# bbc/turingcodec

Hardware: AMD Instinct MI355X
Metric: encoded fps (havoc hot path, primitive-batch throughput: one picture's primitive calls per frame as whole-frame batches; (higher is better)
Workload: dtype u8

## Files before the change

### turingcodec_amd/csrc/kernels_rdoq.hip

```cpp
#include "common.h"
#include "rdoq_work.h"

#include <cstdlib>

namespace havoc_gpu {

#ifdef HAVOC_RDOQ_TIMING
__device__ unsigned long long g_rdoqTiming[32];
struct RdoqTimer
{
    unsigned long long acc[16] = {}, last = __builtin_readcyclecounter();
    __device__ __forceinline__ void mark(int k)
    {
        const unsigned long long now = __builtin_readcyclecounter();
        acc[k] += now - last;
        last = now;
    }
    __device__ __forceinline__ void flush(int lane, int base)
    {
        if (lane != 0) return;
        for (int k = 0; k < 16; ++k)
            if (acc[k]) atomicAdd(&g_rdoqTiming[base + k], acc[k]);
    }
};
#define RT_DECL RdoqTimer rt
#define RT_MARK(k) rt.mark(k)
#define RT_PARAM , RdoqTimer &rt
#define RT_ARG , rt
#define RT_FLUSH(lane, base) rt.flush(lane, base)
#else
#define RT_DECL
#define RT_MARK(k)
#define RT_PARAM
#define RT_ARG
#define RT_FLUSH(lane, base)
#endif

namespace {

__device__ const int32_t kEntropyBits[128] = {
    0x07b23, 0x085f9, 0x074a0, 0x08cbc, 0x06ee4, 0x09354, 0x067f4, 0x09c1b, 0x060b0, 0x0a62a, 0x05a9c, 0x0af5b, 0x0548d, 0x0b955, 0x04f56, 0x0c2a9,
    0x04a87, 0x0cbf7, 0x045d6, 0x0d5c3, 0x04144, 0x0e01b, 0x03d88, 0x0e937, 0x039e0, 0x0f2cd, 0x03663, 0x0fc9e, 0x03347, 0x10600, 0x03050, 0x10f95,
    0x02d4d, 0x11a02, 0x02ad3, 0x12333, 0x0286e, 0x12cad, 0x02604, 0x136df, 0x02425, 0x13f48, 0x021f4, 0x149c4, 0x0203e, 0x1527b, 0x01e4d, 0x15d00,
    0x01c99, 0x166de, 0x01b18, 0x17017, 0x019a5, 0x17988, 0x01841, 0x18327, 0x016df, 0x18d50, 0x015d9, 0x19547, 0x0147c, 0x1a083, 0x0138e, 0x1a8a3,
    0x01251, 0x1b418, 0x01166, 0x1bd27, 0x01068, 0x1c77b, 0x00f7f, 0x1d18e, 0x00eda, 0x1d91a, 0x00e19, 0x1e254, 0x00d4f, 0x1ec9a, 0x00c90, 0x1f6e0,
    0x00c01, 0x1fef8, 0x00b5f, 0x208b1, 0x00ab6, 0x21362, 0x00a15, 0x21e46, 0x00988, 0x2285d, 0x00934, 0x22ea8, 0x008a8, 0x239b2, 0x0081d, 0x24577,
    0x007c9, 0x24ce6, 0x00763, 0x25663, 0x00710, 0x25e8f, 0x006a0, 0x26a26, 0x00672, 0x26f23, 0x005e8, 0x27ef8, 0x005ba, 0x284b5, 0x0055e, 0x29057,
    0x0050c, 0x29bab, 0x004c1, 0x2a674, 0x004a7, 0x2aa5e, 0x0046f, 0x2b32f, 0x0041f, 0x2c0ad, 0x003e7, 0x2ca8d, 0x003ba, 0x2d323, 0x0010c, 0x3bfbb };

typedef short s16x2v __attribute__((ext_vector_type(2)));
typedef unsigned short u16x2v __attribute__((ext_vector_type(2)));

static_assert(sizeof(havoc_mi355x_rdoq_job) == sizeof(RdoqJob), "rdoq job layout");

struct Block
{
    const uint8_t *states;
    const int32_t *bits;
    const int32_t *lastBits;
    int stateStride, lastStride, lastLen;
    int64_t lambda;
    int distShift;
    int quantScale, quantShift, invScale, invShift, invOffset;
    int cIdx, scanIdx;
    uint64_t scan4;
    int64_t csbfZero[2], csbfOne[2];
    int64_t cbfZero, cbfOne;
    const uint32_t *clsTab;
};

struct LevelState { int ctxSet, c1, nG1, nG2, rice; };

__device__ __forceinline__ int32_t bitsOf(const Block &b, int ctx, int bin) { return b.bits[(b.states[ctx * b.stateStride] >> 1) ^ bin]; }
template <class T>
__device__ __forceinline__ T pick(bool c, T a, T b) { return c ? a : b; }

__device__ __forceinline__ int baseLevel(const LevelState &s) { return pick(s.nG1 < 8, 2 + (int)(s.nG2 < 1), 1); }
__device__ __forceinline__ int clip16(int v) { return min(max(v, -32768), 32767); }

__device__ __forceinline__ void diagXy(int size, int pos, int &x, int &y)
{
    for (int d = 0;; ++d)
    {
        const int lo = d < size ? 0 : d - size + 1, hi = d < size ? d : size - 1, len = hi - lo + 1;
        if (pos < len) { x = lo + pos; y = d - x; return; }
        pos -= len;
    }
}
__device__ __forceinline__ void scanXy(int size, int scanIdx, int pos, int &x, int &y)
{
    if (scanIdx == 1) { x = pos & (size - 1); y = pos / size; }
    else if (scanIdx == 2) { x = pos / size; y = pos & (size - 1); }
    else diagXy(size, pos, x, y);
}
__host__ __device__ constexpr uint64_t scan4Nibbles(int scanIdx)
{
    uint64_t v = 0;
    int i = 0;
    if (scanIdx == 0)
    {
        for (int d = 0; d < 7; ++d)
            for (int x = 0; x <= d; ++x)
                if (x < 4 && d - x < 4) { v |= (uint64_t)(x | (d - x) << 2) << (4 * i); ++i; }
    }
    else
        for (; i < 16; ++i) v |= (uint64_t)(scanIdx == 1 ? i : (i >> 2) | (i & 3) << 2) << (4 * i);
    return v;
}

template <int GW>
__device__ __forceinline__ void toScanOrder(int scanIdx, uint64_t &m, uint64_t &m2, uint64_t &m3)
{
    if (GW == 1 || scanIdx == 1) return;
    uint64_t a = 0, b = 0, c = 0;
    int x = 0, y = 0;
    for (int g = 0; g < GW * GW; ++g)
    {
        const int p = y * GW + x;
        a |= ((m >> p) & 1) << g;
        b |= ((m2 >> p) & 1) << g;
        c |= ((m3 >> p) & 1) << g;
        if (scanIdx == 2)
        {
            if (++y == GW) { y = 0; ++x; }
        }
        else
// ... 200 lines not shown
            z = bitsOf(b, ctx, 0);
            one = bitsOf(b, ctx, 1);
            zeroBits += pick(inside & !nonZero, z, 0);
        }
        else
        {
            const bool is1 = (cls1 >> i) & 1, is2 = (cls2 >> i) & 1, isD = i == 0 && dcGroup;
            z = pick(isD, zcD, pick(is1, zc1, pick(is2, zc2, zc0)));
            one = pick(isD, ocD, pick(is1, oc1, pick(is2, oc2, oc0)));
        }
        sh.rec.kept[nib][lane] = 0;
        const int32_t upZero = (int32_t)((uint32_t)factor * (uint32_t)-(scaled >> (b.quantShift - 8))) + (1 << 15) + one - z;
        sh.rec.costUp[i][lane] = pick(inside, upZero, 1 << 15);
    }
    const uint32_t zeroMask = active & ~nzMask;
    if (LOG2 > 2)
        zeroBits = zc0 * __popc(zeroMask & cls0) + zc1 * __popc(zeroMask & cls1) + zc2 * __popc(zeroMask & cls2) + zcD * __popc(zeroMask & clsD);
    const int64_t sumSq = ((int64_t)sumAllHi << 16) + sumAll;
    r.dist0 = sumSq << b.distShift;

    RT_MARK(4);
    int nonZeroAbovePos0 = 0;
    int64_t gSig = 0, gSigPos0 = 0, gCoded = 0, gDist0 = 0, costB = 0, distB = 0, qB = 0;
    uint32_t c1At = 0x55555555u;
    uint32_t keptMask = 0, oddMask = 0;
    for (uint32_t m = nzMask; m;)
    {
        const int i = 31 - __clz((int)m);
        m ^= 1u << i;
        const int nib = (int)(b.scan4 >> (4 * i)) & 15, x = (gx << 2) + (nib & 3), y = (gy << 2) + (nib >> 2);
        const int a = abs((int)sh.coef[nib][lane]);
        const int64_t dist0 = (int64_t)(a * a) << b.distShift;
        const int sp = g * 16 + i;
        const int scaled = a * b.quantScale;
        const int level = (scaled + rnd) >> b.quantShift;
        const bool first = sp == firstPos;
        int32_t z0, z1, aboveBits;
        if (LOG2 == 2)
        {
            const uint32_t pk = reinterpret_cast<const uint32_t (*)[64]>(sh.rec.costDown)[i][lane];
            const int sc = (int)(pk >> 25);
            aboveBits = (int32_t)(pk & 0x1ffffff);
            z0 = bitsOf(b, sc, 0);
            z1 = bitsOf(b, sc, 1);
        }
        else
        {
            const bool is1 = (cls1 >> i) & 1, is2 = (cls2 >> i) & 1, isD = (clsD >> i) & 1;
            z0 = pick(isD, zcD, pick(is1, zc1, pick(is2, zc2, zc0)));
            z1 = pick(isD, ocD, pick(is1, oc1, pick(is2, oc2, oc0)));
            const uint32_t above = zeroMask & ~((2u << i) - 1);
            aboveBits = zc0 * __popc(above & cls0) + zc1 * __popc(above & cls1) + zc2 * __popc(above & cls2);
        }
        const int64_t zerosAbove = b.lambda * aboveBits;
        const int32_t sigZero = pick(first, 0, z0), sigOneBits = pick(first, 0, z1);
        fb.g1zero = pick4(aux.g1zero, st.c1);
        fb.g1one = pick4(g1one, st.c1);

        const bool droppable = !first && level < 3;
        const int64_t sigOne = b.lambda * sigOneBits, dropSig = b.lambda * sigZero;
        const int lower = level - 1;
        const int32_t err1 = a - clip16((clip16(level) * b.invScale + b.invOffset) >> b.invShift);
        const int32_t err2 = a - clip16((clip16(lower) * b.invScale + b.invOffset) >> b.invShift);
        const int64_t cost1 = ((int64_t)(int32_t)((uint32_t)err1 * (uint32_t)err1) << b.distShift) + b.lambda * levelBits(level, st, fb) + sigOne;
        const int64_t cost2If = ((int64_t)(int32_t)((uint32_t)err2 * (uint32_t)err2) << b.distShift) + b.lambda * levelBits(lower, st, fb) + sigOne;
        const int64_t cost2 = pick(lower >= 1, cost2If, (int64_t)INT64_MAX);
        const int64_t dropCost = dist0 + dropSig;
        int64_t costCoded = pick(droppable, dropCost, (int64_t)INT64_MAX), costSig = pick(droppable, dropSig, (int64_t)0);
        int kept = 0;
        const bool take1 = cost1 < costCoded;
        kept = pick(take1, level, kept);
        costSig = pick(take1, sigOne, costSig);
        costCoded = pick(take1, cost1, costCoded);
        const bool take2 = cost2 < costCoded;
        kept = pick(take2, lower, kept);
        costSig = pick(take2, sigOne, costSig);
        costCoded = pick(take2, cost2, costCoded);

        costB += costCoded;
        distB += dist0;
        const int du = (scaled - (kept << b.quantShift)) >> (b.quantShift - 8), sigDelta = sigOneBits - sigZero;
        const int stored = (int16_t)kept;
        const int now = levelRate(kept, st, fb);
        const int upKept = factor * -du + levelRate(kept + 1, st, fb) - now;
        const int upZero = factor * -abs(du) + (1 << 15) + sigDelta;
        sh.rec.kept[nib][lane] = (int16_t)kept;
        keptMask |= (uint32_t)(stored != 0) << i;
        oddMask |= (uint32_t)(stored & 1) << i;
        sh.rec.costUp[i][lane] = pick(kept > 0, upKept, upZero);
        const int lastOne = (1 << 15) + sigDelta;
        sh.rec.costDown[i][lane] = factor * du + levelRate(kept - 1, st, fb) - now - pick(kept == 1, lastOne, 0);

        const bool grow = (kept >= baseLevel(st)) & (kept > 3 * (1 << st.rice));
        st.rice = pick(grow, min(st.rice + 1, 4), st.rice);
        st.nG1 += kept >= 1;
        st.nG2 += kept > 1;
        const bool step = (st.c1 < 3) & (st.c1 > 0) & (kept != 0);
        st.c1 = pick(kept > 1, 0, pick(step, st.c1 + 1, st.c1));
        {
            const uint32_t below = (1u << (2 * i)) - 1;
            c1At = (c1At & ~below) | ((0x55555555u * (uint32_t)st.c1) & below);
        }
        gSig += costSig;
        gSigPos0 = pick(i == 0, costSig, gSigPos0);
        const int64_t codedPart = costCoded - costSig;
        gCoded += pick(stored != 0, codedPart, (int64_t)0);
        gDist0 += pick(stored != 0, dist0, (int64_t)0);
        nonZeroAbovePos0 += (stored != 0) & (i != 0);
        const int lx = lastPrefixLength(x), ly = lastPrefixLength(y);
        const int32_t rate = b.lastBits[(b.scanIdx == 2 ? ly : lx) * b.lastStride] + b.lastBits[(b.lastLen + (b.scanIdx == 2 ? lx : ly)) * b.lastStride];
        const int64_t total = qB - zerosAbove + b.lambda * rate - costSig;
        const bool better = (stored != 0) & !r.localStop & (total < r.localBest);
        r.localBest = pick(better, total, r.localBest);
        r.localPos = pick(better, sp, r.localPos);
        r.localOr = pick(better, 0, r.localOr) | stored;
        r.groupOr |= stored;
        r.localStop |= stored > 1;
        const int64_t keptGain = dist0 - costCoded, zeroGain = -costSig;
        qB += pick(stored != 0, keptGain, zeroGain);
    }
    RT_MARK(5);
    aux.c1At = c1At;
    aux.keptMask = keptMask;
    aux.oddMask = oddMask;
    aux.negScan = negScan;
    aux.negRaster = negRaster;
    const int64_t zeroCost = b.lambda * zeroBits;
    r.cost = (r.dist0 - distB) + zeroCost + costB;
    r.q = qB - zeroCost;
    gSig += zeroCost;
    if (!(nzMask & 1))
        gSigPos0 = LOG2 == 2 ? zeroCost - b.lambda * (int32_t)(reinterpret_cast<const uint32_t (*)[64]>(sh.rec.costDown)[0][lane] & 0x1ffffff) : b.lambda * pick(dcGroup, zcD, pick((bool)(cls1 & 1), zc1, pick((bool)(cls2 & 1), zc2, zc0)));
    r.carry = st.c1 == 0;
    const bool dc = g == 0, any = keptMask != 0, inner = any & !dc & (g < firstGroup);
    const int64_t zero = pick(neighbours != 0, b.csbfZero[1], b.csbfZero[0]), one = pick(neighbours != 0, b.csbfOne[1], b.csbfOne[0]);
    const int64_t implied = pick(inner & (nonZeroAbovePos0 == 0), gSigPos0, (int64_t)0);
    const int64_t sigLeft = gSig - implied, allZero = zero + gDist0 - gCoded - sigLeft;
    const bool dropped = inner & (allZero < one), empty = !any & !dc;
    const int64_t innerCost = pick(dropped, allZero, one) - implied, emptyCost = zero - gSig;
    r.cost += pick(empty, emptyCost, pick(inner, innerCost, (int64_t)0));
    r.sigCost = pick(empty | dropped, zero, pick(inner, one, (int64_t)0));
    r.coded = dc | (any & !dropped);
    RT_MARK(6);
    return r;
}

__device__ __forceinline__ void hideSignsWalk(WalkShared &sh, int lane, const Block &b, bool lastGroup, const SdhAux &aux, uint32_t keptMask)
{
    const int first = max(__ffs((int)keptMask) - 1, 0), last = keptMask ? 31 - __clz((int)keptMask) : 0;
    const int signbit = (int)(aux.negScan >> first) & 1;
    const bool needed = (keptMask != 0) & (last - first >= 4) & (signbit != (__popc(aux.oddMask & keptMask) & 1));
    if (__ballot(needed) == 0) return;
    const int top = lastGroup ? last : 15;
    int minCost = INT32_MAX, minIdx = 0, finalChange = 0;
#pragma unroll
    for (int i = 15; i >= 0; --i)
    {
        const bool isKept = (keptMask >> i) & 1;
        const int mag = (uint16_t)sh.rec.kept[(int)(b.scan4 >> (4 * i)) & 15][lane];
        const int up = sh.rec.costUp[i][lane];
        const int downRaw = pick(isKept, sh.rec.costDown[i][lane], 0);
        const int down = downRaw - pick(lastGroup & (last == i) & (mag == 1), 4 << 15, 0);
        const bool upBetter = up < down;
        const int costKept = pick(upBetter, up, pick((i == first) & (mag == 1), INT32_MAX, down));
        const int g1 = pick((aux.active >> i) & 1, pick4(aux.g1zero, (int)(aux.c1At >> (2 * i)) & 3), 0);
        const int costZero = pick((i < first) & (((int)(aux.negScan >> i) & 1) != signbit), INT32_MAX, up + g1);
        const int cost = pick(isKept, costKept, costZero), change = pick(isKept & !upBetter, -1, 1);
        const bool better = (i <= top) & (cost < minCost);
        minCost = pick(better, cost, minCost);
        finalChange = pick(better, change, finalChange);
        minIdx = pick(better, i, minIdx);
    }
    if (!needed) return;
    const int nib = (int)(b.scan4 >> (4 * minIdx)) & 15;
    const int mag = (uint16_t)sh.rec.kept[nib][lane], negative = (int)(aux.negScan >> minIdx) & 1;
    if ((!negative && mag == 32767) || (negative && mag == 32768)) finalChange = -1;
    sh.rec.kept[nib][lane] = (int16_t)(mag + finalChange);
}

struct ScanShared
{
    int32_t srcOff[64], dstOff[64], nzThreshold[64], gt1Threshold[64], gt2Threshold[64];
    uint64_t mask[64], mask2[64], mask3[64];
    int64_t sumSq[64];
};
// ... 62 lines not shown
}

constexpr int kScanSteps = 8;
template <int LOG2>
__global__ __launch_bounds__(64) void k_rdoq_scan(int16_t *__restrict__ dstAll, const int16_t *__restrict__ srcAll, const RdoqJob *__restrict__ jobs, int njobs,
                                                  RdoqWork *__restrict__ work, int withHist)
{
    constexpr int perWg = kScanSteps * (64 / (((1 << LOG2) * (1 << LOG2)) >> 4));
    __shared__ ScanShared sc;
    __shared__ uint32_t hist[kBins];
    const int lane = threadIdx.x, first = blockIdx.x * perWg, blk = first + lane;
    RdoqInfo *info = reinterpret_cast<RdoqInfo *>(reinterpret_cast<char *>(work) + rdoqInfoOffset());
    for (int k = lane; k < kBins; k += 64) hist[k] = 0;
    scanBlocks<LOG2>(sc, dstAll, srcAll, jobs, njobs, first, kScanSteps);
    if (lane < perWg && blk < njobs)
    {
        RdoqInfo r;
        r.mask = sc.mask[lane];
        r.mask2 = sc.mask2[lane];
        r.mask3 = sc.mask3[lane];
        r.sumSq = sc.sumSq[lane];
        info[blk] = r;
        atomicAdd(&hist[groupsToWalk(r.mask)], 1u);
        if (jobs[blk].scan_idx != 0) atomicAdd(&hist[kBins - 1], 1u);
    }
    __syncthreads();
    if (!withHist) return;
    for (int k = lane; k < kBins - 1; k += 64)
        if (hist[k]) atomicAdd(&work->hist[k], hist[k]);
    if (lane == 0 && hist[kBins - 1]) atomicAdd(&work->otherScans, hist[kBins - 1]);
}

__global__ __launch_bounds__(256) void k_rdoq_hist(const RdoqJob *__restrict__ jobs, int njobs, RdoqWork *__restrict__ work)
{
    __shared__ uint32_t hist[kBins];
    const RdoqInfo *info = reinterpret_cast<const RdoqInfo *>(reinterpret_cast<const char *>(work) + rdoqInfoOffset());
    const int t = threadIdx.x, blk = blockIdx.x * 256 + t;
    if (t < kBins) hist[t] = 0;
    __syncthreads();
    if (blk < njobs)
    {
        atomicAdd(&hist[groupsToWalk(info[blk].mask)], 1u);
        if (jobs[blk].scan_idx != 0) atomicAdd(&hist[kBins - 1], 1u);
    }
    __syncthreads();
    if (t < kBins - 1 && hist[t]) atomicAdd(&work->hist[t], hist[t]);
    if (t == kBins - 1 && hist[t]) atomicAdd(&work->otherScans, hist[t]);
}

template <int LOG2>
__global__ __launch_bounds__(256) void k_rdoq_order(const RdoqJob *__restrict__ jobs, int njobs, RdoqWork *__restrict__ work)
{
    __shared__ uint32_t count[kBins], base[kBins];
    RdoqInfo *info = reinterpret_cast<RdoqInfo *>(reinterpret_cast<char *>(work) + rdoqInfoOffset());
    uint32_t *order = reinterpret_cast<uint32_t *>(info + njobs);
    const int t = threadIdx.x, blk = blockIdx.x * 256 + t;
    if (t < kBins) count[t] = 0;
    __syncthreads();
    int bin = 0;
    uint32_t rank = 0;
    if (blk < njobs)
    {
        RdoqInfo v = info[blk];
        bin = groupsToWalk(v.mask);
        rank = atomicAdd(&count[bin], 1u);
        toScanOrder<(1 << LOG2) / 4>(jobs[blk].scan_idx, v.mask, v.mask2, v.mask3);
        info[blk] = v;
    }
    __syncthreads();
    __shared__ uint32_t histAll[kBins];
    if (t < kBins) histAll[t] = work->hist[t];
    __syncthreads();
    if (t < kBins && count[t])
    {
        uint32_t before = 0;
        for (int k = t + 1; k < kBins - 1; ++k) before += histAll[k];
        base[t] = before + atomicAdd(&work->cursor[t], count[t]);
    }
    __syncthreads();
    if (blk < njobs) order[base[bin] + rank] = (uint32_t)blk;
}

template <int LOG2>
struct LaneBlock
{
    static constexpr int size = 1 << LOG2, G = (size * size) >> 4, gw = size >> 2;
    Block b;
    const uint8_t *rasterOf;
    const uint8_t *scanOf;
    const int16_t *src;
    int16_t *dst;
    int distShift;

    template <class BT>
    __device__ __forceinline__ void stageIn(WalkShared &sh, BT &bt, int lane, int slot, int sub, int per, const RdoqJob &job,
                                            const uint8_t *__restrict__ statesAll, int bitDepth, const int16_t *__restrict__ srcAll, int16_t *__restrict__ dstAll)
    {
        constexpr int SLOTS = BT::slots;
        static_assert(BT::nlen == 2 * LOG2, "prefix lengths of a coordinate");
        sh.bits[lane] = kEntropyBits[lane];
        sh.bits[64 + lane] = kEntropyBits[64 + lane];
        if (BT::ldsStates)
        {
            const uint32_t *st = reinterpret_cast<const uint32_t *>(statesAll + (long)job.ctx_index * HAVOC_RDOQ_CTX_BYTES);
            for (int k = sub; k < HAVOC_RDOQ_CTX_BYTES / 4; k += per)
            {
                const uint32_t v = st[k];
                bt.states[4 * k][slot] = (uint8_t)v;
                bt.states[4 * k + 1][slot] = (uint8_t)(v >> 8);
                bt.states[4 * k + 2][slot] = (uint8_t)(v >> 16);
                bt.states[4 * k + 3][slot] = (uint8_t)(v >> 24);
            }
        }
        if (lane < G)
            for (int t = 0; t < 3; ++t)
            {
                int x = 0, y = 0;
                if (G > 1) scanXy(gw, t, lane, x, y);
                sh.rasterOf[t][lane] = (uint8_t)(y * gw + x);
                sh.scanOf[t][y * gw + x] = (uint8_t)lane;
            }
        if (lane < 12)
        {
            const int t = lane >> 2, nb = lane & 3;
            const uint64_t sc = t == 0 ? scan4Nibbles(0) : (t == 1 ? scan4Nibbles(1) : scan4Nibbles(2));
            const uint32_t pat = nb == 0 ? sigPattern(0) : nb == 1 ? sigPattern(1) : nb == 2 ? sigPattern(2) : sigPattern(3);
            uint32_t one = 0, two = 0;
            for (int i = 0; i < 16; ++i)
            {
                const uint32_t inc = (pat >> (2 * ((int)(sc >> (4 * i)) & 15))) & 3;
                one |= (uint32_t)(inc == 1) << i;
                two |= (uint32_t)(inc == 2) << i;
            }
            sh.clsScan[t][nb] = one | two << 16;
        }
        __syncthreads();

        b.states = BT::ldsStates ? &bt.states[0][slot] : statesAll + (long)job.ctx_index * HAVOC_RDOQ_CTX_BYTES;
        b.stateStride = BT::ldsStates ? SLOTS : 1;
        b.lastBits = &bt.lastBits[0][0][slot];
        b.lastStride = SLOTS;
        b.lastLen = BT::nlen;
        b.bits = sh.bits;
        b.lambda = job.lambda_q16;
        const int transformShift = 15 - bitDepth - LOG2;
        distShift = 15 - 2 * transformShift - 2 * (bitDepth - 8) + 16;
        b.distShift = distShift;
        b.invShift = 6 - transformShift;
        b.invOffset = 1 << (b.invShift - 1);
        b.quantScale = job.quant_scale;
        b.quantShift = job.quant_shift;
        b.invScale = job.inv_scale;
        b.cIdx = job.c_idx;
        b.scanIdx = job.scan_idx;
        b.scan4 = job.scan_idx == 0 ? scan4Nibbles(0) : (job.scan_idx == 1 ? scan4Nibbles(1) : scan4Nibbles(2));
        rasterOf = sh.rasterOf[job.scan_idx < 3 ? job.scan_idx : 0];
        scanOf = sh.scanOf[job.scan_idx < 3 ? job.scan_idx : 0];
        b.clsTab = sh.clsScan[job.scan_idx < 3 ? job.scan_idx : 0];
        src = srcAll + job.src_off;
        dst = dstAll + job.dst_off;
        if (G > 1)
        {
            const int csbf = HAVOC_RDOQ_CTX_CSBF + (b.cIdx ? 2 : 0);
            b.csbfZero[0] = b.lambda * bitsOf(b, csbf, 0);
            b.csbfOne[0] = b.lambda * bitsOf(b, csbf, 1);
            b.csbfZero[1] = b.lambda * bitsOf(b, csbf + 1, 0);
            b.csbfOne[1] = b.lambda * bitsOf(b, csbf + 1, 1);
        }
        else
            b.csbfZero[0] = b.csbfZero[1] = b.csbfOne[0] = b.csbfOne[1] = 0;
        {
            const int cbfCtx = (!job.is_intra && b.cIdx == 0) ? HAVOC_RDOQ_CTX_ROOT_CBF : (b.cIdx == 0 ? HAVOC_RDOQ_CTX_CBF_LUMA + 1 : HAVOC_RDOQ_CTX_CBF_CHROMA);
            b.cbfZero = b.lambda * bitsOf(b, cbfCtx, 0);
            b.cbfOne = b.lambda * bitsOf(b, cbfCtx, 1);
        }
        if (sub == 0)
            for (int axis = 0; axis < 2; ++axis)
            {
                const int base = axis ? HAVOC_RDOQ_CTX_LAST_Y : HAVOC_RDOQ_CTX_LAST_X;
                const int offset = b.cIdx ? 15 : 3 * (LOG2 - 2) + ((LOG2 - 1) >> 2), shift = b.cIdx ? LOG2 - 2 : (LOG2 + 1) >> 2;
                int32_t ones = 0;
                for (int len = 0; len < BT::nlen; ++len)
                {
                    const int ctx = base + min(max((len >> shift) + offset, 0), 17);
                    bt.lastBits[axis][len][slot] = ones + (len < 9 ? bitsOf(b, ctx, 0) : 0) + (len > 3 ? 32768 * ((len - 2) >> 1) : 0);
                    if (len < 9) ones += bitsOf(b, ctx, 1);
                }
            }
        __syncthreads();
    }
    __device__ __forceinline__ void loadGroup(WalkShared &sh, int lane, int gx, int gy) const
    {
        for (int r = 0; r < 4; ++r)
        {
            const u32x2 v = ld8(src + ((gy << 2) + r) * size + (gx << 2));
            sh.coef[4 * r][lane] = (int16_t)v.x;
            sh.coef[4 * r + 1][lane] = (int16_t)(v.x >> 16);
            sh.coef[4 * r + 2][lane] = (int16_t)v.y;
            sh.coef[4 * r + 3][lane] = (int16_t)(v.y >> 16);
        }
    }
    __device__ __forceinline__ void finishGroup(WalkShared &sh, int lane, bool sdh, const SdhAux &aux, int g, int lastIdx, bool lastGroup, int gx, int gy) const
    {
        uint32_t keptMask = aux.keptMask;
        if (lastGroup)
        {
            const int n = lastIdx - g * 16;
            const uint32_t stay = n >= 16 ? 0xffffu : (1u << n) - 1;
            for (int i = 0; i < 16; ++i)
                if (!((stay >> i) & 1)) sh.rec.kept[(int)(b.scan4 >> (4 * i)) & 15][lane] = 0;
            keptMask &= stay;
        }
        if (sdh) hideSignsWalk(sh, lane, b, lastGroup, aux, keptMask);
        for (int r = 0; r < 4; ++r)
        {
            int v[4];
            for (int k = 0; k < 4; ++k)
            {
                const int mag = (uint16_t)sh.rec.kept[4 * r + k][lane];
                v[k] = ((aux.negRaster >> (4 * r + k)) & 1) ? -mag : mag;
            }
            u32x2 o;
            o.x = (uint32_t)(uint16_t)v[0] | (uint32_t)(uint16_t)v[1] << 16;
            o.y = (uint32_t)(uint16_t)v[2] | (uint32_t)(uint16_t)v[3] << 16;
            st8(dst + ((gy << 2) + r) * size + (gx << 2), o);
        }
    }
// ... 46 lines not shown
        rel -= zero;
    }
    __device__ __forceinline__ void walkedGroup(const WalkResult &r, int g, int p, int carryIn, const uint8_t *scanOf, int gw)
    {
        costTu += r.cost;
        walkedDist0 += r.dist0;
        coded |= (uint64_t)r.coded << p;
        codedScan |= (uint64_t)r.coded << g;
        if (gw > 1)
        {
            const int gx = p & (gw - 1), gy = p / gw;
            const bool left = r.coded && gx > 0, above = r.coded && gy > 0;
            nbrScan |= (uint64_t)left << scanOf[left ? p - 1 : 0];
            nbrScan |= (uint64_t)above << scanOf[above ? p - gw : 0];
        }
        carries |= (uint64_t)carryIn << g;
        rel -= r.sigCost;
        if (r.coded)
        {
            if (!stopped && r.localPos >= 0 && rel + r.localBest < bestRel)
            {
                bestRel = rel + r.localBest;
                bestPos = r.localPos;
                orSince = r.localOr;
            }
            else
                orSince |= r.groupOr;
            stopped |= r.localStop;
            rel += r.q;
        }
    }
};

enum WalkSource { kInKernel, kSorted, kJobOrder };
template <int LOG2, bool LDS_STATES>
struct WalkLds
{
    __attribute__((aligned(16))) unsigned char walkMem[sizeof(WalkShared) > sizeof(ScanShared) ? sizeof(WalkShared) : sizeof(ScanShared)];
    BlockTables<64, 2 * LOG2, LDS_STATES> bt;
};
template <int LOG2, WalkSource SOURCE, bool LDS_STATES>
__device__ __forceinline__ void walkBody(WalkLds<LOG2, LDS_STATES> &lds, int wg, int16_t *__restrict__ dstAll, const int16_t *__restrict__ srcAll,
                                         const uint8_t *__restrict__ statesAll, const RdoqJob *__restrict__ jobs, int njobs, int32_t *__restrict__ cbfOut, int bitDepth,
                                         const RdoqWork *__restrict__ work, int onlyOther, int masksByScan = 0)
{
    constexpr bool SORTED = SOURCE == kSorted;
    typedef LaneBlock<LOG2> LB;
    constexpr int G = LB::G, gw = LB::gw;
    unsigned char *walkMem = lds.walkMem;
    WalkShared &sh = *reinterpret_cast<WalkShared *>(walkMem);
    BlockTables<64, 2 * LOG2, LDS_STATES> &bt = lds.bt;
    if (SORTED && onlyOther && work->otherScans == 0) return;
    const RdoqInfo *infoAll = reinterpret_cast<const RdoqInfo *>(reinterpret_cast<const char *>(work) + rdoqInfoOffset());
    const uint32_t *order = reinterpret_cast<const uint32_t *>(infoAll + njobs);
    const int lane = threadIdx.x, slot = wg * 64 + lane;
    bool valid = slot < njobs;
    const int blk = valid ? (SORTED ? (int)order[slot] : slot) : 0;
    const RdoqJob job = jobs[blk];
    if (onlyOther && job.scan_idx == 0) valid = false;
    if (SOURCE == kJobOrder && onlyOther && __ballot(valid) == 0) return;
    RdoqInfo info;
    if (SORTED)
        info = infoAll[blk];
    else if (SOURCE == kJobOrder)
    {
        info = infoAll[blk];
        if (!masksByScan) toScanOrder<gw>(job.scan_idx, info.mask, info.mask2, info.mask3);
    }
    else
    {
        ScanShared &sc = *reinterpret_cast<ScanShared *>(walkMem);
        scanBlocks<LOG2>(sc, dstAll, srcAll, jobs, njobs, wg * 64, G);
        info.mask = sc.mask[lane];
        info.mask2 = info.mask3 = 0;
        info.sumSq = sc.sumSq[lane];
        toScanOrder<gw>(job.scan_idx, info.mask, info.mask2, info.mask3);
        __syncthreads();
    }
    RT_DECL;
    LB lb;
    lb.stageIn(sh, bt, lane, lane, 0, 1, job, statesAll, bitDepth, srcAll, dstAll);
    RT_MARK(0);
    const Block &b = lb.b;
    const uint8_t *rasterOf = lb.rasterOf;
    SdhAux aux;

    uint64_t nz = valid ? info.mask : 0;
    int g = nz ? 63 - __clzll((long long)nz) : -1;
    const int firstGroup = g;
    int firstPos = -1;
    if (firstGroup >= 0)
    {
        const int p = rasterOf[firstGroup];
        lb.loadGroup(sh, lane, p & (gw - 1), p / gw);
        firstPos = firstGroup * 16 + lb.firstInGroup(sh, lane);
        nz |= 1;
    }

    WalkState ws;
    int carry = 0;
    while (__ballot(g >= 0) != 0)
    {
        if (g >= 0)
        {
            const int p = rasterOf[g], gx = p & (gw - 1), gy = p / gw;
            RT_MARK(2);
            lb.loadGroup(sh, lane, gx, gy);
            const WalkResult r = walkGroup<LOG2>(b, sh, lane, g, gx, gy, firstPos, LB::caseOf(ws.coded, gx, gy, carry), job.sdh_factor, aux RT_ARG);
            ws.walkedGroup(r, g, p, carry, lb.scanOf, gw);
            RT_MARK(8);
            if (r.coded && g != 0) lb.finishGroup(sh, lane, job.sdh, aux, g, 1 << 30, false, gx, gy);
            RT_MARK(9);
            const uint64_t below = nz & ((1ull << g) - 1);
            const int next = below ? 63 - __clzll((long long)below) : -1;
            if (G > 1) ws.zeroGroups(((1ull << g) - 1) & ~((2ull << max(next, 0)) - 1) & ~below, b);
            carry = next == g - 1 ? r.carry : 0;
            g = next;
        }
    }
    RT_MARK(2);
// ... 15 lines not shown
        {
            const int p = rasterOf[lastGroup], gx = p & (gw - 1), gy = p / gw;
            lb.loadGroup(sh, lane, gx, gy);
            walkGroup<LOG2>(b, sh, lane, lastGroup, gx, gy, firstPos, LB::caseOf(ws.coded, gx, gy, (int)(ws.carries >> lastGroup) & 1), job.sdh_factor, aux RT_ARG);
            lb.finishGroup(sh, lane, job.sdh, aux, lastGroup, lastIdx, true, gx, gy);
        }
    }
    if (valid) cbfOut[blk] = cbf;
    RT_MARK(11);
    RT_FLUSH(lane, 0);
#ifdef HAVOC_RDOQ_TIMING
    if (lane == 0) atomicAdd(&g_rdoqTiming[15], 1ull);
#endif
}

template <int LOG2, WalkSource SOURCE, bool LDS_STATES>
__global__ __launch_bounds__(64, 2) void k_rdoq_walk(int16_t *__restrict__ dstAll, const int16_t *__restrict__ srcAll, const uint8_t *__restrict__ statesAll,
                                                  const RdoqJob *__restrict__ jobs, int njobs, int32_t *__restrict__ cbfOut, int bitDepth,
                                                  const RdoqWork *__restrict__ work, int onlyOther)
{
    __shared__ WalkLds<LOG2, LDS_STATES> lds;
    walkBody<LOG2, SOURCE, LDS_STATES>(lds, blockIdx.x, dstAll, srcAll, statesAll, jobs, njobs, cbfOut, bitDepth, work, onlyOther);
}

struct DiagExchange
{
    int64_t cost[64], sigCost[64], dist0[64], q[64], localBest[64];
    int32_t localPos[64], localOr[64], groupOr[64];
    int32_t flags[64];
};

template <int LOG2, int LPB>
__global__ __launch_bounds__(64, 2) void k_rdoq_diag(int16_t *__restrict__ dstAll, const int16_t *__restrict__ srcAll, const uint8_t *__restrict__ statesAll,
                                                  const RdoqJob *__restrict__ jobs, int njobs, int32_t *__restrict__ cbfOut, int bitDepth,
                                                  const RdoqWork *__restrict__ work, int sorted, int diagWgs)
{
    struct DiagLds
    {
        WalkShared sh;
        BlockTables<64 / LPB, 2 * LOG2, true> bt;
        DiagExchange ex;
    };
    __shared__ union { DiagLds d; WalkLds<LOG2, false> w; } mem;
    if ((int)blockIdx.x >= diagWgs)
    {
        walkBody<LOG2, kJobOrder, false>(mem.w, blockIdx.x - diagWgs, dstAll, srcAll, statesAll, jobs, njobs, cbfOut, bitDepth, work, 1, sorted);
        return;
    }
    typedef LaneBlock<LOG2> LB;
    constexpr int G = LB::G, gw = LB::gw, ND = 2 * gw - 1;
    WalkShared &sh = mem.d.sh;
    BlockTables<64 / LPB, 2 * LOG2, true> &bt = mem.d.bt;
    DiagExchange &ex = mem.d.ex;
    const RdoqInfo *infoAll = reinterpret_cast<const RdoqInfo *>(reinterpret_cast<const char *>(work) + rdoqInfoOffset());
    const uint32_t *order = reinterpret_cast<const uint32_t *>(infoAll + njobs);
    const int lane = threadIdx.x, k = lane & (LPB - 1), lane0 = lane & ~(LPB - 1), slot = blockIdx.x * (64 / LPB) + lane / LPB;
    bool valid = slot < njobs;
    const int blk = valid ? (sorted ? (int)order[slot] : slot) : 0;
    const RdoqJob job = jobs[blk];
    valid = valid && job.scan_idx == 0;
    RdoqInfo info = infoAll[blk];
    RT_DECL;
    LB lb;
    lb.stageIn(sh, bt, lane, lane / LPB, k, LPB, job, statesAll, bitDepth, srcAll, dstAll);
    RT_MARK(0);
    const Block &b = lb.b;
    const uint8_t *rasterOf = lb.rasterOf;
    SdhAux aux;
    if (!sorted)
    {
        uint64_t m[3] = {0, 0, 0};
        for (int g = k; g < G; g += LPB)
        {
            const int p = rasterOf[g];
            m[0] |= ((info.mask >> p) & 1) << g;
            m[1] |= ((info.mask2 >> p) & 1) << g;
            m[2] |= ((info.mask3 >> p) & 1) << g;
        }
#pragma unroll
        for (int q = 0; q < 3; ++q)
        {
            uint32_t lo = (uint32_t)m[q], hi = (uint32_t)(m[q] >> 32);
#pragma unroll
            for (int d = 1; d < LPB; d <<= 1)
            {
                lo |= (uint32_t)__shfl_xor((int)lo, d, kWave);
                hi |= (uint32_t)__shfl_xor((int)hi, d, kWave);
            }
            m[q] = (uint64_t)hi << 32 | lo;
        }
        info.mask = m[0];
        info.mask2 = m[1];
        info.mask3 = m[2];
    }

    uint64_t walkScan = valid ? info.mask : 0;
    const uint64_t sureScan = valid ? info.mask3 : 0, openScan = valid ? info.mask2 & ~info.mask3 : 0;
    const int firstGroup = walkScan ? 63 - __clzll((long long)walkScan) : -1;
    int firstPos = -1;
    if (firstGroup >= 0)
    {
        const int p = rasterOf[firstGroup];
        lb.loadGroup(sh, lane, p & (gw - 1), p / gw);
        firstPos = firstGroup * 16 + lb.firstInGroup(sh, lane);
        walkScan |= 1;
    }

    WalkState ws;
// ... 104 lines not shown
    __syncthreads();
            RT_MARK(10);
        }
        if (firstGroup >= start) hopZeros(start);
    }

    if (valid && k == 0)
    {
        int cbf = 0;
        if (firstPos >= 0)
        {
            const int lastIdx = lb.lastIndex(job.is_intra, info.sumSq, ws.walkedDist0, ws.costTu, ws.bestRel, ws.bestPos);
            cbf = lastIdx ? ws.orSince : 0;
            const int lastGroup = (lastIdx - 1) >> 4;
            for (uint64_t m = ws.codedScan & ~((2ull << max(lastGroup, 0)) - 1); m;)
            {
                const int g = 63 - __clzll((long long)m);
                m ^= 1ull << g;
                lb.clearGroup(rasterOf[g]);
            }
            if (lastGroup >= 0) lb.finishGroup(sh, lane, job.sdh, aux, 0, lastGroup == 0 ? lastIdx : 1 << 30, lastGroup == 0, 0, 0);
            if (lastGroup > 0 && (lastIdx & 15 || job.sdh))
            {
                const int p = rasterOf[lastGroup], gx = p & (gw - 1), gy = p / gw;
                lb.loadGroup(sh, lane, gx, gy);
                walkGroup<LOG2>(b, sh, lane, lastGroup, gx, gy, firstPos, LB::caseOf(ws.coded, gx, gy, (int)(ws.carries >> lastGroup) & 1), job.sdh_factor, aux RT_ARG);
                lb.finishGroup(sh, lane, job.sdh, aux, lastGroup, lastIdx, true, gx, gy);
            }
        }
        cbfOut[blk] = cbf;
    }
    RT_MARK(11);
    RT_FLUSH(lane, 16);
#ifdef HAVOC_RDOQ_TIMING
    if (lane == 0) atomicAdd(&g_rdoqTiming[31], 1ull);
#endif
}
}

#ifdef HAVOC_RDOQ_TIMING
extern "C" __attribute__((visibility("default"))) int havoc_mi355x_debug_rdoq_timing(unsigned long long *out, int reset)
{
    if (hipDeviceSynchronize() != hipSuccess) return -1;
    if (out && hipMemcpyFromSymbol(out, HIP_SYMBOL(g_rdoqTiming), sizeof(g_rdoqTiming)) != hipSuccess) return -2;
    if (reset)
    {
        unsigned long long z[32] = {};
        if (hipMemcpyToSymbol(HIP_SYMBOL(g_rdoqTiming), z, sizeof(z)) != hipSuccess) return -3;
    }
    return 0;
}
#endif

size_t rdoq_workspace_bytes(int njobs) { return rdoqInfoOffset() + (size_t)max(njobs, 0) * (sizeof(RdoqInfo) + sizeof(uint32_t)) + 64; }

static int envInt(const char *name, int otherwise) { const char *v = getenv(name); return v ? atoi(v) : otherwise; }

static int diagLanes(int log2, int njobs)
{
    static const int diagEnv = envInt("HAVOC_RDOQ_DIAG", 0), diag16Env = envInt("HAVOC_RDOQ_DIAG16", 0);
    return log2 == 5 ? (diagEnv == 0 || njobs > 16 * 1024 ? 0 : (diagEnv == 8 ? 8 : 4)) : (diag16Env == 0 ? 0 : (diag16Env == 8 ? 8 : 4));
}
static bool inJobOrder(int log2, int njobs)
{
    static const int sortEnv = envInt("HAVOC_RDOQ_SORT", 1);
    if (sortEnv == 1 || (sortEnv == 2 && log2 == 4) || (sortEnv == 3 && log2 == 5)) return false;
    const int diag = diagLanes(log2, njobs);
    const long waves = diag ? ((long)njobs * diag + 63) / 64 : ((long)njobs + 63) / 64;
    return waves <= 1024;
}

template <int LOG2>
static void launchDiag(hipStream_t st, int lpb, int16_t *dst, const int16_t *src, const uint8_t *states, const RdoqJob *j, int njobs, int32_t *cbf, int bitDepth,
                       RdoqWork *work, int sorted)
{
    const int wgd = (njobs + 64 / lpb - 1) / (64 / lpb), tail = (njobs + 63) / 64;
    if (lpb == 4) hipLaunchKernelGGL((k_rdoq_diag<LOG2, 4>), dim3(wgd + tail), dim3(64), 0, st, dst, src, states, j, njobs, cbf, bitDepth, work, sorted, wgd);
    else hipLaunchKernelGGL((k_rdoq_diag<LOG2, 8>), dim3(wgd + tail), dim3(64), 0, st, dst, src, states, j, njobs, cbf, bitDepth, work, sorted, wgd);
}

static hipError_t rdoq_order_and_walk(hipStream_t st, int bitDepth, int log2, int16_t *dst, const int16_t *src, const uint8_t *states, const RdoqJob *j, int njobs,
                                      int32_t *cbf, RdoqWork *work, bool jobOrder)
{
    const int wgs = (njobs + 63) / 64;
    const int diag = diagLanes(log2, njobs);
    if (jobOrder)
    {
        if (diag)
        {
            if (log2 == 5) launchDiag<5>(st, diag, dst, src, states, j, njobs, cbf, bitDepth, work, 0);
            else launchDiag<4>(st, diag, dst, src, states, j, njobs, cbf, bitDepth, work, 0);
        }
        else if (log2 == 4) hipLaunchKernelGGL((k_rdoq_walk<4, kJobOrder, false>), dim3(wgs), dim3(64), 0, st, dst, src, states, j, njobs, cbf, bitDepth, work, 0);
        else hipLaunchKernelGGL((k_rdoq_walk<5, kJobOrder, false>), dim3(wgs), dim3(64), 0, st, dst, src, states, j, njobs, cbf, bitDepth, work, 0);
        return hipGetLastError();
    }
    if (log2 == 4) hipLaunchKernelGGL(k_rdoq_order<4>, dim3((njobs + 255) / 256), dim3(256), 0, st, j, njobs, work);
    else hipLaunchKernelGGL(k_rdoq_order<5>, dim3((njobs + 255) / 256), dim3(256), 0, st, j, njobs, work);
    if (diag)
    {
        if (log2 == 5) launchDiag<5>(st, diag, dst, src, states, j, njobs, cbf, bitDepth, work, 1);
        else launchDiag<4>(st, diag, dst, src, states, j, njobs, cbf, bitDepth, work, 1);
    }
    else if (log2 == 4) hipLaunchKernelGGL((k_rdoq_walk<4, kSorted, true>), dim3(wgs), dim3(64), 0, st, dst, src, states, j, njobs, cbf, bitDepth, work, 0);
    else hipLaunchKernelGGL((k_rdoq_walk<5, kSorted, true>), dim3(wgs), dim3(64), 0, st, dst, src, states, j, njobs, cbf, bitDepth, work, 0);
    return hipGetLastError();
}
// ... 60 lines not shown
```

### turingcodec_amd/csrc/rdoq_work.h

```cpp
#pragma once

#include <cstddef>
#include <cstdint>

namespace havoc_gpu {

struct RdoqJob
{
    int32_t dst_off, src_off, quant_scale, quant_shift, inv_scale, lambda_q16, sdh_factor, ctx_index;
    uint8_t c_idx, scan_idx, is_intra, sdh;
    int32_t reserved[3];
};
static_assert(sizeof(RdoqJob) == 48, "rdoq job layout");

struct RdoqInfo { uint64_t mask, mask2, mask3; int64_t sumSq; };
constexpr int kBins = 66;
struct RdoqWork
{
    uint32_t hist[kBins], cursor[kBins];
    uint32_t otherScans, pad[3];
};
__host__ __device__ inline size_t rdoqInfoOffset() { return (sizeof(RdoqWork) + 15) & ~size_t(15); }
__device__ __forceinline__ int groupsToWalk(uint64_t mask) { return mask ? __popcll(mask | 1) : 0; }

__device__ __forceinline__ void rdoqThresholds(int quantScale, int quantShift, uint32_t (&thr)[3])
{
    const uint32_t half = 1u << (quantShift - 1), scale = (uint32_t)(quantScale > 1 ? quantScale : 1);
    thr[0] = (half + scale - 1) / scale;
    thr[1] = (3 * half + scale - 1) / scale;
    thr[2] = (5 * half + scale - 1) / scale;
}

}
```

Baseline: 1554.

## Store RDOQ lambda as 32-bit and keep scan-order masks in a separate buffer

Lambda is narrowed to a 32-bit field, and each cost is built by adding the bit counts first and then doing one 32x64 multiply via a helper. This replaces several 64-bit multiplies per coefficient. The order kernel now writes scan-order masks into a new byScan region instead of overwriting the raster-order info, and the walk kernels read from it. This lets job-order paths skip the toScanOrder conversion when masks are already in scan order. The cost is a larger workspace, and the merged additions could overflow 32 bits if bit sums grow large.

```diff
diff --git a/turingcodec_amd/csrc/kernels_rdoq.hip b/turingcodec_amd/csrc/kernels_rdoq.hip
--- a/turingcodec_amd/csrc/kernels_rdoq.hip
+++ b/turingcodec_amd/csrc/kernels_rdoq.hip
@@ -59,7 +59,7 @@
     const int32_t *bits;
     const int32_t *lastBits;
     int stateStride, lastStride, lastLen;
-    int64_t lambda;
+    int32_t lambda;
     int distShift;
     int quantScale, quantShift, invScale, invShift, invOffset;
     int cIdx, scanIdx;
@@ -72,6 +72,7 @@
 struct LevelState { int ctxSet, c1, nG1, nG2, rice; };
 
 __device__ __forceinline__ int32_t bitsOf(const Block &b, int ctx, int bin) { return b.bits[(b.states[ctx * b.stateStride] >> 1) ^ bin]; }
+__device__ __forceinline__ int64_t lambdaBits(const Block &b, int32_t bits) { return (int64_t)b.lambda * bits; }
 template <class T>
 __device__ __forceinline__ T pick(bool c, T a, T b) { return c ? a : b; }
 
@@ -378,18 +379,17 @@
             const uint32_t above = zeroMask & ~((2u << i) - 1);
             aboveBits = zc0 * __popc(above & cls0) + zc1 * __popc(above & cls1) + zc2 * __popc(above & cls2);
         }
-        const int64_t zerosAbove = b.lambda * aboveBits;
         const int32_t sigZero = pick(first, 0, z0), sigOneBits = pick(first, 0, z1);
         fb.g1zero = pick4(aux.g1zero, st.c1);
         fb.g1one = pick4(g1one, st.c1);
 
         const bool droppable = !first && level < 3;
-        const int64_t sigOne = b.lambda * sigOneBits, dropSig = b.lambda * sigZero;
+        const int64_t sigOne = lambdaBits(b, sigOneBits), dropSig = lambdaBits(b, sigZero);
         const int lower = level - 1;
         const int32_t err1 = a - clip16((clip16(level) * b.invScale + b.invOffset) >> b.invShift);
         const int32_t err2 = a - clip16((clip16(lower) * b.invScale + b.invOffset) >> b.invShift);
-        const int64_t cost1 = ((int64_t)(int32_t)((uint32_t)err1 * (uint32_t)err1) << b.distShift) + b.lambda * levelBits(level, st, fb) + sigOne;
-        const int64_t cost2If = ((int64_t)(int32_t)((uint32_t)err2 * (uint32_t)err2) << b.distShift) + b.lambda * levelBits(lower, st, fb) + sigOne;
+        const int64_t cost1 = ((int64_t)(int32_t)((uint32_t)err1 * (uint32_t)err1) << b.distShift) + lambdaBits(b, levelBits(level, st, fb) + sigOneBits);
+        const int64_t cost2If = ((int64_t)(int32_t)((uint32_t)err2 * (uint32_t)err2) << b.distShift) + lambdaBits(b, levelBits(lower, st, fb) + sigOneBits);
         const int64_t cost2 = pick(lower >= 1, cost2If, (int64_t)INT64_MAX);
         const int64_t dropCost = dist0 + dropSig;
         int64_t costCoded = pick(droppable, dropCost, (int64_t)INT64_MAX), costSig = pick(droppable, dropSig, (int64_t)0);
@@ -435,7 +435,7 @@
         nonZeroAbovePos0 += (stored != 0) & (i != 0);
         const int lx = lastPrefixLength(x), ly = lastPrefixLength(y);
         const int32_t rate = b.lastBits[(b.scanIdx == 2 ? ly : lx) * b.lastStride] + b.lastBits[(b.lastLen + (b.scanIdx == 2 ? lx : ly)) * b.lastStride];
-        const int64_t total = qB - zerosAbove + b.lambda * rate - costSig;
+        const int64_t total = qB + lambdaBits(b, rate - aboveBits) - costSig;
         const bool better = (stored != 0) & !r.localStop & (total < r.localBest);
         r.localBest = pick(better, total, r.localBest);
         r.localPos = pick(better, sp, r.localPos);
@@ -451,12 +451,12 @@
     aux.oddMask = oddMask;
     aux.negScan = negScan;
     aux.negRaster = negRaster;
-    const int64_t zeroCost = b.lambda * zeroBits;
+    const int64_t zeroCost = lambdaBits(b, zeroBits);
     r.cost = (r.dist0 - distB) + zeroCost + costB;
     r.q = qB - zeroCost;
     gSig += zeroCost;
     if (!(nzMask & 1))
-        gSigPos0 = LOG2 == 2 ? zeroCost - b.lambda * (int32_t)(reinterpret_cast<const uint32_t (*)[64]>(sh.rec.costDown)[0][lane] & 0x1ffffff) : b.lambda * pick(dcGroup, zcD, pick((bool)(cls1 & 1), zc1, pick((bool)(cls2 & 1), zc2, zc0)));
+        gSigPos0 = LOG2 == 2 ? zeroCost - lambdaBits(b, (int32_t)(reinterpret_cast<const uint32_t (*)[64]>(sh.rec.costDown)[0][lane] & 0x1ffffff)) : lambdaBits(b, pick(dcGroup, zcD, pick((bool)(cls1 & 1), zc1, pick((bool)(cls2 & 1), zc2, zc0))));
     r.carry = st.c1 == 0;
     const bool dc = g == 0, any = keptMask != 0, inner = any & !dc & (g < firstGroup);
     const int64_t zero = pick(neighbours != 0, b.csbfZero[1], b.csbfZero[0]), one = pick(neighbours != 0, b.csbfOne[1], b.csbfOne[0]);
@@ -625,8 +625,9 @@
 __global__ __launch_bounds__(256) void k_rdoq_order(const RdoqJob *__restrict__ jobs, int njobs, RdoqWork *__restrict__ work)
 {
     __shared__ uint32_t count[kBins], base[kBins];
-    RdoqInfo *info = reinterpret_cast<RdoqInfo *>(reinterpret_cast<char *>(work) + rdoqInfoOffset());
-    uint32_t *order = reinterpret_cast<uint32_t *>(info + njobs);
+    const RdoqInfo *info = reinterpret_cast<const RdoqInfo *>(reinterpret_cast<const char *>(work) + rdoqInfoOffset());
+    uint32_t *order = reinterpret_cast<uint32_t *>(reinterpret_cast<char *>(work) + rdoqOrderOffset(njobs));
+    RdoqInfo *byScan = reinterpret_cast<RdoqInfo *>(reinterpret_cast<char *>(work) + rdoqByScanOffset(njobs));
     const int t = threadIdx.x, blk = blockIdx.x * 256 + t;
     if (t < kBins) count[t] = 0;
     __syncthreads();
@@ -638,7 +639,7 @@
         bin = groupsToWalk(v.mask);
         rank = atomicAdd(&count[bin], 1u);
         toScanOrder<(1 << LOG2) / 4>(jobs[blk].scan_idx, v.mask, v.mask2, v.mask3);
-        info[blk] = v;
+        byScan[blk] = v;
     }
     __syncthreads();
     __shared__ uint32_t histAll[kBins];
@@ -735,17 +736,17 @@
         if (G > 1)
         {
             const int csbf = HAVOC_RDOQ_CTX_CSBF + (b.cIdx ? 2 : 0);
-            b.csbfZero[0] = b.lambda * bitsOf(b, csbf, 0);
-            b.csbfOne[0] = b.lambda * bitsOf(b, csbf, 1);
-            b.csbfZero[1] = b.lambda * bitsOf(b, csbf + 1, 0);
-            b.csbfOne[1] = b.lambda * bitsOf(b, csbf + 1, 1);
+            b.csbfZero[0] = lambdaBits(b, bitsOf(b, csbf, 0));
+            b.csbfOne[0] = lambdaBits(b, bitsOf(b, csbf, 1));
+            b.csbfZero[1] = lambdaBits(b, bitsOf(b, csbf + 1, 0));
+            b.csbfOne[1] = lambdaBits(b, bitsOf(b, csbf + 1, 1));
         }
         else
             b.csbfZero[0] = b.csbfZero[1] = b.csbfOne[0] = b.csbfOne[1] = 0;
         {
             const int cbfCtx = (!job.is_intra && b.cIdx == 0) ? HAVOC_RDOQ_CTX_ROOT_CBF : (b.cIdx == 0 ? HAVOC_RDOQ_CTX_CBF_LUMA + 1 : HAVOC_RDOQ_CTX_CBF_CHROMA);
-            b.cbfZero = b.lambda * bitsOf(b, cbfCtx, 0);
-            b.cbfOne = b.lambda * bitsOf(b, cbfCtx, 1);
+            b.cbfZero = lambdaBits(b, bitsOf(b, cbfCtx, 0));
+            b.cbfOne = lambdaBits(b, bitsOf(b, cbfCtx, 1));
         }
         if (sub == 0)
             for (int axis = 0; axis < 2; ++axis)
@@ -898,7 +899,8 @@
     BlockTables<64, 2 * LOG2, LDS_STATES> &bt = lds.bt;
     if (SORTED && onlyOther && work->otherScans == 0) return;
     const RdoqInfo *infoAll = reinterpret_cast<const RdoqInfo *>(reinterpret_cast<const char *>(work) + rdoqInfoOffset());
-    const uint32_t *order = reinterpret_cast<const uint32_t *>(infoAll + njobs);
+    const RdoqInfo *byScan = reinterpret_cast<const RdoqInfo *>(reinterpret_cast<const char *>(work) + rdoqByScanOffset(njobs));
+    const uint32_t *order = reinterpret_cast<const uint32_t *>(reinterpret_cast<const char *>(work) + rdoqOrderOffset(njobs));
     const int lane = threadIdx.x, slot = wg * 64 + lane;
     bool valid = slot < njobs;
     const int blk = valid ? (SORTED ? (int)order[slot] : slot) : 0;
@@ -907,11 +909,15 @@
     if (SOURCE == kJobOrder && onlyOther && __ballot(valid) == 0) return;
     RdoqInfo info;
     if (SORTED)
-        info = infoAll[blk];
+        info = byScan[blk];
     else if (SOURCE == kJobOrder)
     {
-        info = infoAll[blk];
-        if (!masksByScan) toScanOrder<gw>(job.scan_idx, info.mask, info.mask2, info.mask3);
+        if (masksByScan) info = byScan[blk];
+        else
+        {
+            info = infoAll[blk];
+            toScanOrder<gw>(job.scan_idx, info.mask, info.mask2, info.mask3);
+        }
     }
     else
     {
@@ -1033,8 +1039,8 @@
     WalkShared &sh = mem.d.sh;
     BlockTables<64 / LPB, 2 * LOG2, true> &bt = mem.d.bt;
     DiagExchange &ex = mem.d.ex;
-    const RdoqInfo *infoAll = reinterpret_cast<const RdoqInfo *>(reinterpret_cast<const char *>(work) + rdoqInfoOffset());
-    const uint32_t *order = reinterpret_cast<const uint32_t *>(infoAll + njobs);
+    const RdoqInfo *infoAll = reinterpret_cast<const RdoqInfo *>(reinterpret_cast<const char *>(work) + (sorted ? rdoqByScanOffset(njobs) : rdoqInfoOffset()));
+    const uint32_t *order = reinterpret_cast<const uint32_t *>(reinterpret_cast<const char *>(work) + rdoqOrderOffset(njobs));
     const int lane = threadIdx.x, k = lane & (LPB - 1), lane0 = lane & ~(LPB - 1), slot = blockIdx.x * (64 / LPB) + lane / LPB;
     bool valid = slot < njobs;
     const int blk = valid ? (sorted ? (int)order[slot] : slot) : 0;
@@ -1245,7 +1251,7 @@
 }
 #endif
 
-size_t rdoq_workspace_bytes(int njobs) { return rdoqInfoOffset() + (size_t)max(njobs, 0) * (sizeof(RdoqInfo) + sizeof(uint32_t)) + 64; }
+size_t rdoq_workspace_bytes(int njobs) { njobs = max(njobs, 0); return rdoqByScanOffset(njobs) + (size_t)njobs * sizeof(RdoqInfo) + 64; }
 
 static int envInt(const char *name, int otherwise) { const char *v = getenv(name); return v ? atoi(v) : otherwise; }
 
diff --git a/turingcodec_amd/csrc/rdoq_work.h b/turingcodec_amd/csrc/rdoq_work.h
--- a/turingcodec_amd/csrc/rdoq_work.h
+++ b/turingcodec_amd/csrc/rdoq_work.h
@@ -21,6 +21,8 @@
     uint32_t otherScans, pad[3];
 };
 __host__ __device__ inline size_t rdoqInfoOffset() { return (sizeof(RdoqWork) + 15) & ~size_t(15); }
+__host__ __device__ inline size_t rdoqOrderOffset(int njobs) { return rdoqInfoOffset() + (size_t)njobs * sizeof(RdoqInfo); }
+__host__ __device__ inline size_t rdoqByScanOffset(int njobs) { return (rdoqOrderOffset(njobs) + (size_t)njobs * sizeof(uint32_t) + 15) & ~size_t(15); }
 __device__ __forceinline__ int groupsToWalk(uint64_t mask) { return mask ? __popcll(mask | 1) : 0; }
 
 __device__ __forceinline__ void rdoqThresholds(int quantScale, int quantShift, uint32_t (&thr)[3])
```

Result: no change. 1556 (median of 6 runs) (+0.1%).
